# aifoundry-org/MHAQ

Measured on AMD Instinct MI355X. Metric: qat_images_per_sec, higher is better.
Workload: dtype f32; 1 GPU; ResNet-18 ImageNet-1k QAT step, AEWGS weights per-channel + STE activations, Sym-KL distillation from FP teacher, RAdam, synthetic 224x224, channels_last memory format; per_gpu_batch=250, global_batch=250, parallelism=dp1, sync_batchnorm=False, weight_backward_groups=3, cudnn_benchmark=False

## Files before the change

### mhaq_amd/csrc/torch_binding.cpp

```cpp
#include <torch/extension.h>
#include <torch/version.h>
#include <torch/csrc/autograd/custom_function.h>

#include <c10/hip/HIPCachingAllocator.h>
#include <c10/hip/HIPGraphsC10Utils.h>
#include <c10/hip/HIPStream.h>
#include <c10/core/DeviceGuard.h>
#include <dlfcn.h>

#include <algorithm>
#include <atomic>
#include <chrono>
#include <cstring>
#include <map>
#include <memory>
#include <mutex>
#include <string>
#include <unordered_map>
#include <vector>

#include "../../include/mhaq_fq.h"

namespace py = pybind11;
using at::Tensor;
// ... 756 lines not shown
    variable_list out(9);
    if (!grads[0].defined()) return out;
    TORCH_CHECK(!(at::GradMode::is_enabled() && grads[0].requires_grad()),
                "bn_pool_train: the node is once-differentiable (no double backward)");
    at::NoGradGuard no_grad;
    auto saved = ctx->get_saved_variables();
    const Tensor &x = saved[0], &w = saved[1], &mean = saved[2], &invstd = saved[3], &code = saved[4];
    const std::array<bool, 3> mask = {ctx->needs_input_grad(0), ctx->needs_input_grad(1), ctx->needs_input_grad(2)};
    Tensor g = grads[0].scalar_type() == at::kFloat ? grads[0] : grads[0].to(at::kFloat);
    if (g.sizes() != code.sizes() || g.strides() != code.strides()) {
      Tensor dense = at::empty_like(code, code.options().dtype(at::kFloat));
      dense.copy_(g);
      g = dense;
    }
    return bn_hip_backward(9, x, g, code, w, mean, invstd, mask);
  }
};

Tensor bn_pool_train(const Tensor& x, const std::optional<Tensor>& w, const std::optional<Tensor>& b,
                     const std::optional<Tensor>& running_mean, const std::optional<Tensor>& running_var, double momentum,
                     double eps, bool cudnn_enabled, bool hip_forward) {
  TORCH_CHECK(w.has_value() && w->defined() && b.has_value() && b->defined(),
              "bn_pool_train: an affine BatchNorm (weight and bias) is required");
  MHAQ_ON_DEVICE_OF(x);
  const bool hipf = hip_forward && bn_hip_forward_eligible(x, *w, *b, opt_tensor(running_mean), opt_tensor(running_var));
  if (!(bn_hip_eligible(x, *w) && x.scalar_type() == at::kFloat && x.numel() / x.size(1) < (1ll << 31)))
    return at::max_pool2d(BatchNormTrainFn::apply(x, w, b, running_mean, running_var, momentum, eps, cudnn_enabled,
                                                  false, hipf),
                          {3, 3}, {2, 2}, {1, 1});
  need_lib();
  return BatchNormPoolTrainFn::apply(x, *w, *b, running_mean, running_var, momentum, eps, cudnn_enabled, hipf);
}

struct Pre {
  bool has = false;
  Tensor wq, s, zp, mx, lwq;
};

PyObject* g_allreduce_avg = nullptr;
std::atomic<bool> g_dist_active{false};

void allreduce_avg(const Tensor& t) {
  py::gil_scoped_acquire gil;
  if (!g_allreduce_avg) throw MhaqError("AEWGS statistics exchange requested but no all-reduce is installed");
  py::reinterpret_borrow<py::object>(g_allreduce_avg)(t);
}

class WeightLayerFn : public torch::autograd::Function<WeightLayerFn> {
 public:
  static variable_list forward(AutogradContext* ctx, const Tensor& w, const Tensor& log_s, int64_t method,
                               const std::optional<Tensor>& r_sign, bool zp_grad, const Pre& pre, int64_t rank,
                               bool distributed) {
    const int64_t co = w.size(0), row = co ? w.numel() / co : 0;
    Tensor wq, s, zp, mx, lwq;
    if (pre.has) {
      wq = pre.wq; s = pre.s; zp = pre.zp; mx = pre.mx; lwq = pre.lwq;
    } else {
      wq = at::empty_like(w);
      Tensor aux = at::empty({4, co}, w.options());
      s = aux.select(0, 0); zp = aux.select(0, 1); mx = aux.select(0, 2); lwq = aux.select(0, 3);
      check(A.mhaq_fq_wlayer_fwd(fptr(w), fptr_mut(wq), fptr(log_s), co, row, fptr_mut(s), fptr_mut(zp), fptr_mut(mx),
                                 fptr_mut(lwq), cur_stream(w)),
            "mhaq_fq_wlayer_fwd");
    }
    weight_save_ctx(ctx, {w, s, zp, mx}, r_sign, method, rank, log_s);
    ctx->saved_data["dist"] = distributed;
    if (!zp_grad) ctx->mark_non_differentiable({s, zp});
    return {wq, zp, s, lwq};
  }

  static variable_list backward(AutogradContext* ctx, variable_list grads) {
    auto saved = ctx->get_saved_variables();
    const Tensor &w = saved[0], &s = saved[1], &zp = saved[2], &mx = saved[3];
    const bool has_r = saved.size() > 4;
    const int64_t method = ctx->saved_data["method"].toInt();
    Tensor G = grads[0].defined() ? like_layout(grads[0], w) : at::zeros_like(w);
    Tensor gzp_extra = grads[1].defined() ? grads[1].contiguous() : Tensor();
    Tensor g_lwq = grads[3].defined() ? grads[3].contiguous() : Tensor();
    const int64_t co = w.size(0), row = co ? w.numel() / co : 0;
    Tensor stats;
    if (method == MHAQ_FQ_AEWGS && ctx->saved_data["dist"].toBool()) {
      stats = at::empty({3, co}, w.options());
      check(A.mhaq_fq_pc_aewgs_stats(fptr(w), fptr(G), fptr(s), fptr(zp), co, row, fptr_mut(stats), cur_stream(w)),
            "mhaq_fq_pc_aewgs_stats");
      allreduce_avg(stats);
    }
    Tensor gw = at::empty_like(w);
    Tensor gls = at::empty({co}, w.options());
    const Draw d = draw_signs(has_r, method, ctx->saved_data["rank"].toInt(), w);
    check(A.mhaq_fq_wlayer_bwd(fptr(w), fptr(G), fptr_mut(gw), fptr_mut(gls), fptr(s), fptr(zp), fptr(mx),
                               fptr_or_null(g_lwq), co, row, (int)method, fptr_or_null(stats), fptr_or_null(gzp_extra),
                               saved_sign(saved, 4), d.seed, d.offset, d.offset_dev, cur_stream(w)),
          "mhaq_fq_wlayer_bwd");
    if (grads[2].defined())
      gls = gls + at::mul(at::mul(grads[2].reshape({co}), s), 0.69314718055994531);
    variable_list out(8);
    out[0] = gw;
    out[1] = ls_view(ctx, gls);
    return out;
  }
};

std::tuple<Tensor, Tensor, Tensor, Tensor> weight_layer(const Tensor& w_in, const Tensor& log_s_in, int64_t method,
                                                        const std::optional<Tensor>& r_sign, bool zp_grad,
                                                        const std::optional<std::vector<Tensor>>& pre, int64_t rank) {
  need_lib();
// ... 9 lines not shown
  if (pre.has_value()) {
    TORCH_CHECK(pre->size() >= 5, "weight_layer: pre = (wq, s, zp, mx, lwq[, s and zp in the published shape])");
    p.has = true;
    p.wq = (*pre)[0]; p.s = (*pre)[1]; p.zp = (*pre)[2]; p.mx = (*pre)[3]; p.lwq = (*pre)[4];
  }
  auto out = WeightLayerFn::apply(w, log_s, method, r_sign, zp_grad, p, rank, g_dist_active.load());
  std::vector<int64_t> shp(w.dim(), 1);
  shp[0] = w.size(0);
  return {out[0], out[1].view(shp), out[2].view(shp), out[3]};
}

std::tuple<Tensor, Tensor, Tensor, Tensor> pt_result(const variable_list& out) {
  const Tensor& aux = out[1];
  return {out[0], aux.select(0, 1), aux.narrow(0, 0, 1), out[2]};
}

class WeightLayerPTFn : public torch::autograd::Function<WeightLayerPTFn> {
 public:
  static variable_list forward(AutogradContext* ctx, const Tensor& w, const Tensor& log_s, int64_t method,
                               const std::optional<Tensor>& r_sign, int64_t rank) {
    Tensor wq = at::empty_like(w);
    Tensor aux = at::empty({4}, w.options());
    check(A.mhaq_fq_wlayer_pt_fwd(fptr(w), fptr_mut(wq), fptr(log_s), w.numel(), fptr_mut(aux), cur_stream(w)),
          "mhaq_fq_wlayer_pt_fwd");
    Tensor lwq = aux.narrow(0, 3, 1).clone();
    weight_save_ctx(ctx, {w, aux}, r_sign, method, rank, log_s);
    ctx->mark_non_differentiable({aux});
    return {wq, aux, lwq};
  }

  static variable_list backward(AutogradContext* ctx, variable_list grads) {
    auto saved = ctx->get_saved_variables();
    const Tensor &w = saved[0], &aux = saved[1];
    const bool has_r = saved.size() > 2;
    const int64_t method = ctx->saved_data["method"].toInt();
    Tensor G = grads[0].defined() ? grads[0].contiguous() : at::zeros_like(w);
    Tensor g_lwq = grads[2].defined() ? grads[2].contiguous() : Tensor();
    Tensor gw = at::empty_like(w);
    Tensor gls = at::empty({1}, w.options());
    const Draw d = draw_signs(has_r, method, ctx->saved_data["rank"].toInt(), w);
    check(A.mhaq_fq_wlayer_pt_bwd(fptr(w), fptr(G), fptr_mut(gw), fptr_mut(gls), fptr(aux), fptr_or_null(g_lwq), w.numel(),
                                  (int)method, saved_sign(saved, 2), d.seed, d.offset, d.offset_dev, cur_stream(w)),
          "mhaq_fq_wlayer_pt_bwd");
    variable_list out(5);
    out[0] = gw;
    out[1] = ls_view(ctx, gls);
    return out;
  }
};

std::tuple<Tensor, Tensor, Tensor, Tensor> weight_layer_pt(const Tensor& w_in, const Tensor& log_s, int64_t method,
                                                           const std::optional<Tensor>& r_sign, int64_t rank) {
  need_lib();
  MHAQ_ON_DEVICE_OF(w_in);
  TORCH_CHECK(w_in.is_cuda() && w_in.scalar_type() == at::kFloat && log_s.is_cuda() &&
                  log_s.scalar_type() == at::kFloat && log_s.numel() == 1,
              "weight_layer_pt: weight and a one-element log_wght_s must be float32 device tensors");
  const Tensor w = w_in.contiguous();
  auto out = WeightLayerPTFn::apply(w, log_s, method, r_sign, rank);
  return pt_result(out);
}

class WeightLayerPTLFn : public torch::autograd::Function<WeightLayerPTLFn> {
 public:
  static variable_list forward(AutogradContext* ctx, const Tensor& w, const Tensor& log_s, int64_t method,
                               const std::optional<Tensor>& r_sign, int64_t rank, bool distributed) {
    Tensor wq = at::empty_like(w);
    Tensor aux = at::empty({7}, w.options());
    const size_t nb = A.mhaq_fq_wlayer_ptl_workspace_bytes(w.numel());
    Tensor ws = at::empty({(int64_t)nb}, w.options().dtype(at::kByte));
    check(A.mhaq_fq_wlayer_ptl_fwd(fptr(w), fptr_mut(wq), fptr(log_s), w.numel(), fptr_mut(aux), ws.mutable_data_ptr(), nb,
                                   cur_stream(w)),
          "mhaq_fq_wlayer_ptl_fwd");
    Tensor lwq = aux.narrow(0, 3, 1).clone();
    weight_save_ctx(ctx, {w, aux}, r_sign, method, rank, log_s);
    ctx->saved_data["dist"] = distributed;
    ctx->mark_non_differentiable({aux});
    return {wq, aux, lwq};
  }

  static variable_list backward(AutogradContext* ctx, variable_list grads) {
    auto saved = ctx->get_saved_variables();
    const Tensor &w = saved[0], &aux = saved[1];
    const bool has_r = saved.size() > 2;
    const int64_t method = ctx->saved_data["method"].toInt();
    Tensor G = grads[0].defined() ? like_layout(grads[0], w) : at::zeros_like(w);
    Tensor g_lwq = grads[2].defined() ? grads[2].contiguous() : Tensor();
    const int64_t n = w.numel();
    void* stream = cur_stream(w);
    Tensor stats;
    int64_t period = 0;
    if (method == MHAQ_FQ_AEWGS) {
      const int64_t co = w.size(0);
      period = n / co;
      stats = at::empty({3, period}, w.options());
      const size_t sb = A.mhaq_fq_pt_aewgs_colstats_workspace_bytes(co, period);
      Tensor sws = sb ? at::empty({(int64_t)sb}, w.options().dtype(at::kByte)) : Tensor();
      check(A.mhaq_fq_pt_aewgs_colstats(fptr(w), fptr(G), co, period, fptr(aux), fptr(aux) + 1, nullptr, nullptr,
                                        fptr_mut(stats), sb ? sws.mutable_data_ptr() : nullptr, sb, stream),
            "mhaq_fq_pt_aewgs_colstats");
      if (ctx->saved_data["dist"].toBool()) allreduce_avg(stats);
    }
    Tensor gw = at::empty_like(w);
    Tensor gls = at::empty({1}, w.options());
    const size_t nb = A.mhaq_fq_wlayer_ptl_workspace_bytes(n);
    Tensor ws = at::empty({(int64_t)nb}, w.options().dtype(at::kByte));
    const Draw d = draw_signs(has_r, method, ctx->saved_data["rank"].toInt(), w);
    check(A.mhaq_fq_wlayer_ptl_bwd(fptr(w), fptr(G), fptr_mut(gw), fptr_mut(gls), fptr(aux), fptr_or_null(g_lwq), n,
                                   (int)method, fptr_or_null(stats), period, saved_sign(saved, 2), d.seed, d.offset,
                                   d.offset_dev, ws.mutable_data_ptr(), nb, stream),
          "mhaq_fq_wlayer_ptl_bwd");
    variable_list out(6);
    out[0] = gw;
    out[1] = ls_view(ctx, gls);
    return out;
  }
// ... 191 lines not shown
    ctx->saved_data["plan"] = plan_id;
    ctx->saved_data["group"] = gi;
    ctx->saved_data["rank"] = rank;
    ctx->saved_data["dist"] = distributed;
    ctx->saved_data["aux"] = p->cur_aux;
    std::vector<std::vector<int64_t>> ls_shapes;
    variable_list ws(tensors.begin(), tensors.begin() + n);
    for (int64_t k = 0; k < n; ++k) ls_shapes.push_back(tensors[n + k].sizes().vec());
    ctx->saved_data["ls_shapes"] = ls_shapes;
    ctx->save_for_backward(ws);
    ctx->set_materialize_grads(false);
    variable_list outs;
    outs.reserve(2 * n);
    for (int64_t k = 0; k < n; ++k) {
      const int64_t i = grp.first + k;
      outs.push_back(at::as_strided(p->cur_wq, ws[k].sizes(), ws[k].strides(), p->elem_off[i]));
    }
    for (int64_t k = 0; k < n; ++k) {
      const int64_t i = grp.first + k;
      outs.push_back(p->cur_aux.select(0, 3).narrow(0, p->chan_off[i], p->co[i]));
    }
    return outs;
  }

  static variable_list backward(AutogradContext* ctx, variable_list grads) {
    auto p = g_plans.get(ctx->saved_data["plan"].toInt());
    std::unique_lock<std::mutex> lk(p->mu);
    Group& grp = p->groups.at(ctx->saved_data["group"].toInt());
    const int64_t n = grp.n;
    auto ws = ctx->get_saved_variables();
    const Tensor aux_all = ctx->saved_data["aux"].toTensor();
    const Tensor& like = aux_all;
    void* stream = cur_stream(like);
    std::vector<Tensor> Gs(n), gl(n);
    for (int64_t k = 0; k < n; ++k) {
      Gs[k] = grads[k].defined() ? like_layout(grads[k], ws[k]) : at::zeros_like(ws[k]);
      if (grads[n + k].defined()) gl[k] = grads[n + k].contiguous();
    }
    if (!grp.pool) grp.pool = std::make_unique<TablePool>(sizeof(mhaq_wlayer_desc) * n, like);
    std::vector<int64_t> key;
    key.reserve(3 * n);
    for (int64_t k = 0; k < n; ++k) key.push_back((int64_t)(uintptr_t)ws[k].const_data_ptr());
    for (int64_t k = 0; k < n; ++k) key.push_back((int64_t)(uintptr_t)Gs[k].const_data_ptr());
    for (int64_t k = 0; k < n; ++k) key.push_back(gl[k].defined() ? (int64_t)(uintptr_t)gl[k].const_data_ptr() : 0);
    const Tensor table = grp.pool->get(key, [&](void* dst) {
      auto* d = static_cast<mhaq_wlayer_desc*>(dst);
      for (int64_t k = 0; k < n; ++k) {
        const int64_t i = grp.first + k;
        d[k] = mhaq_wlayer_desc{fptr(ws[k]), nullptr, fptr(Gs[k]), fptr_or_null(gl[k]), p->co[i], p->row[i],
                                p->elem_off[i] - grp.elem0, p->chan_off[i] - grp.chan0};
      }
    }, stream);
    const auto* descs = static_cast<const mhaq_wlayer_desc*>(table.const_data_ptr());
    const float* aux = fptr(aux_all) + grp.chan0;
    Tensor stats;
    if (grp.method == MHAQ_FQ_AEWGS && ctx->saved_data["dist"].toBool()) {
      stats = at::empty({3, grp.co}, like.options());
      check(A.mhaq_fq_wlayer_aewgs_stats_group(descs, (int)n, grp.co, aux, p->total_co, fptr_mut(stats), stream),
            "mhaq_fq_wlayer_aewgs_stats_group");
      lk.unlock();
      allreduce_avg(stats);
      lk.lock();
    }
    Tensor gw = at::empty({grp.elems}, like.options());
    Tensor gls = at::empty({grp.co}, like.options());
    const Draw d = draw_signs(false, grp.method, ctx->saved_data["rank"].toInt(), like);
// ... 145 lines not shown
    auto h = g_hubs.get(id);
    std::lock_guard<std::mutex> g(h->mu);
    py::dict d;
    d["tables"] = h->tables.entries.size();
    d["captured_tables"] = h->tables.captured();
    d["retired"] = h->retired.size();
    d["pending"] = h->pending.size();
    d["has_table"] = h->last_table.defined();
    int64_t bytes = 0;
    for (auto& w : h->ws) if (w.defined()) bytes += w.numel();
    for (auto& w : h->retired) bytes += w.numel();
    d["workspace_bytes"] = bytes;
    return d;
  });
  m.def("act_layer", &act_layer, py::arg("x"), py::arg("log_act_s"), py::arg("log_act_q"), py::arg("act_b"),
        py::arg("method"), py::arg("r_sign") = py::none(), py::arg("hub") = 0, py::arg("slot") = 0, py::arg("rank") = 0);
  m.def("act_relu_layer", &act_relu_layer, py::arg("z"), py::arg("addend"), py::arg("log_act_s"), py::arg("log_act_q"),
        py::arg("act_b"), py::arg("method"), py::arg("want_act"), py::arg("hub") = 0, py::arg("slot") = 0,
        py::arg("rank") = 0);

  m.def("bn_train", &bn_train, py::arg("x"), py::arg("weight"), py::arg("bias"), py::arg("running_mean"),
        py::arg("running_var"), py::arg("momentum"), py::arg("eps"), py::arg("cudnn_enabled") = true,
        py::arg("x16") = false, py::arg("hip_forward") = false);
  m.def("bn_hip_forwards", []() { return g_bn_hip_forwards.load(); },
        "number of BatchNorm forwards so far (bn_train and bn_pool_train) that ran mhaq_fq_bn_fwd instead of the framework's");

  m.def("bn_hip_backwards", []() { return g_bn_hip_backwards.load(); },
        "number of BatchNorm backwards so far that ran the fp32 HIP kernels instead of the framework's backward");
  m.def("bn_hip_backwards_x16", []() { return g_bn_hip_backwards_x16.load(); },
        "number of BatchNorm backwards so far that ran the 16-bit HIP kernels (mhaq_fq_bn_bwd_x16)");
  m.def("bn_pool_train", &bn_pool_train, py::arg("x"), py::arg("weight"), py::arg("bias"), py::arg("running_mean"),
        py::arg("running_var"), py::arg("momentum"), py::arg("eps"), py::arg("cudnn_enabled") = true,
        py::arg("hip_forward") = false);
  m.def("bn_pool_hip_backwards", []() { return g_bn_pool_hip_backwards.load(); },
        "number of BatchNorm + pool backwards so far that ran mhaq_fq_bn_pool_bwd (the fallback is the two separate nodes)");

  m.def("weight_layer", &weight_layer, py::arg("w"), py::arg("log_wght_s"), py::arg("method"),
        py::arg("r_sign") = py::none(), py::arg("zp_grad") = false, py::arg("pre") = py::none(), py::arg("rank") = 0);
  m.def("weight_layer_pt", &weight_layer_pt, py::arg("w"), py::arg("log_wght_s"), py::arg("method"),
        py::arg("r_sign") = py::none(), py::arg("rank") = 0);
  m.def("weight_layer_ptl", &weight_layer_ptl, py::arg("w"), py::arg("log_wght_s"), py::arg("method"),
        py::arg("r_sign") = py::none(), py::arg("rank") = 0);

  m.def("plan_create", &plan_create);
  m.def("plan_destroy", [](int64_t id) { g_plans.erase(id); });
  m.def("plan_forward", &plan_forward);
  m.def("plan_group_apply", &plan_group_apply);
  m.def("plan_release_captured", [](int64_t id) {
    auto p = g_plans.get(id);
    std::lock_guard<std::mutex> g(p->mu);
    for (auto& grp : p->groups) if (grp.pool) grp.pool->release_captured();
    p->fwd_tables.release_captured();
  });
  m.def("plan_state", [](int64_t id) {
    auto p = g_plans.get(id);
    std::lock_guard<std::mutex> g(p->mu);
    py::dict d;
    d["fwd_tables"] = p->fwd_tables.entries.size();
    py::list pools;
    for (auto& grp : p->groups) {
      py::dict e;
      size_t used = 0, held = 0, size = 0;
      if (grp.pool) {
        size = grp.pool->keys.size();
        for (size_t i = 0; i < size; ++i) { used += grp.pool->used[i]; held += grp.pool->held[i]; }
      }
// ... 10 lines not shown
```

### mhaq_amd/layers.py

```python
from __future__ import annotations

from typing import Tuple

import torch
import torch.nn.functional as F
from torch import inf, nn

from . import ops
from .enums import QNMethod, QScheme
from .gdnsq import Quantizer


def _rnoise_ratio(m):
    if m.rand_noise:
        return m._noise_ratio
    z = getattr(m, "_zero_ratio", None)
    if z is None or z.device != m._noise_ratio.device:
        z = torch.zeros_like(m._noise_ratio)
        m._zero_ratio = z
    return z


class NoisyAct(nn.Module):
    def __init__(
        self,
        init_s=-10,
        init_q=10,
        signed=True,
        noise_ratio=1,
        disable=False,
        qnmethod: QNMethod = QNMethod.STE,
    ) -> None:
        super().__init__()
        self.disable = disable
        self.signed = signed
        zero_point = 0.0 if not signed else -torch.exp2(torch.tensor(init_q - 1).float())
        self._act_b = torch.tensor([zero_point]).float()
        self._log_act_s = torch.tensor([init_s]).float()
        self._log_act_q = torch.tensor([init_q]).float()
        self._noise_ratio = torch.tensor(noise_ratio)
        self.log_act_q = nn.Parameter(self._log_act_q, requires_grad=True)
        self.act_b = nn.Parameter(self._act_b, requires_grad=bool(signed))
        self.log_act_s = nn.Parameter(self._log_act_s, requires_grad=True)
# ... 79 lines not shown
        self.Q.zero_point = self.act_b
        self.Q.min_val = self.act_b
        self.Q.max_val = params[3:4]

    def __getstate__(self):
        state = self.__dict__.copy()
        state.pop("_hub", None)
        return state

    def _forward_unfused_params(self, x):
        s = torch.exp2(self.log_act_s)
        q = torch.exp2(self.log_act_q)
        self.Q.zero_point = self.act_b
        self.Q.min_val = self.act_b
        self.Q.max_val = self.act_b + q - s
        self.Q.scale = s
        if self.training:
            return self.Q.fake_quant(x)
        y, qstats, _ = self.Q.fake_quant_eval(x)
        self.bw = torch.log2(qstats[1] - qstats[0] + 1)
        return y


class _WeightQuantMixin:
    quant_bias = False

    def _quantized_weight(self):
        d = self.__dict__
        self.Q.rnoise_ratio.data = _rnoise_ratio(self)
        weight_p, log_s_p = self.weight, self.log_wght_s
        grad_on = torch.is_grad_enabled()
        key = (weight_p._version, log_s_p._version, grad_on)
        pre = d.get("_precomputed")
        if pre is not None:
            d["_precomputed"] = None
            weight, zp, s, lwq, pkey = pre
            if pkey == key:
                d["_lwq"], d["_lwq_key"] = lwq, key
                self.Q.scale, self.Q.zero_point = s, zp
                return weight, s, zp
        per_channel = self.qscheme == QScheme.PER_CHANNEL
        if per_channel and self.quant_bias:
            weight, zp, s, lwq = ops.fake_quant_weight_layer(weight_p, log_s_p, self.Q.qnmethod, zp_grad=True)
            d["_lwq"], d["_lwq_key"] = lwq, key
        elif per_channel:
            pre = d.get("_pre_fwd")
            group = None
            if pre is not None:
                d["_pre_fwd"] = None
                group = pre[2]
                pre = pre[0] if pre[1] == (key[0], key[1], weight_p.data_ptr()) else None
            if pre is not None and group is not None and grad_on:
                weight, lwq = group[0].take(group[1])
                s, zp = pre[5], pre[6]
            else:
                weight, zp, s, lwq = ops.fake_quant_weight_layer(weight_p, log_s_p, self.Q.qnmethod, pre=pre)
            d["_lwq"], d["_lwq_key"] = lwq, key
        elif ops.small_pt_layer_supported(weight_p, self.Q.qnmethod):
            pre = d.get("_pre_fwd")
            group = None
            if pre is not None:
                d["_pre_fwd"] = None
                ok = pre[1] == (key[0], key[1], weight_p.data_ptr())
                group = pre[2]
                pre = pre[0] if (ok and group is not None and grad_on) else None
            if pre is not None:
                weight, lwq = group[0].take(group[1])
                zp, s = pre[2].reshape(()), pre[1]
            else:
                weight, zp, s, lwq = ops.fake_quant_weight_layer_pt(weight_p, log_s_p, self.Q.qnmethod)
            d["_lwq"], d["_lwq_key"] = lwq, key
        else:
            weight, zp, s, lwq = ops.fake_quant_weight_layer_ptl(weight_p, log_s_p, self.Q.qnmethod)
            d["_lwq"], d["_lwq_key"] = lwq, key
        self.Q.scale = s
        self.Q.zero_point = zp
        return weight, s, zp

    def regulariser_input(self):
        d = self.__dict__
        lwq = d.get("_lwq")
        if lwq is not None and d.get("_lwq_key") == (self.weight._version, self.log_wght_s._version,
                                                     torch.is_grad_enabled()):
            return lwq
        return None

    def __getstate__(self):
        state = self.__dict__.copy()
        for k in ("_pre_fwd", "_precomputed", "_lwq", "_lwq_key", "_zero_ratio"):
            state.pop(k, None)
        return state


class NoisyConv2d(_WeightQuantMixin, nn.Conv2d):
    def __init__(
        self,
        in_channels: int,
        out_channels: int,
        kernel_size: int | Tuple[int, int],
        stride: int | Tuple[int, int] = 1,
        padding: str | int | Tuple[int, int] = 0,
        dilation: int | Tuple[int, int] = 1,
        groups: int = 1,
        bias: bool = True,
        padding_mode: str = "zeros",
        device=None,
        dtype=None,
        qscheme: QScheme = QScheme.PER_TENSOR,
        log_s_init: float = -12,
        rand_noise: bool = False,
        quant_bias: bool = False,
        qnmethod: QNMethod = QNMethod.AEWGS,
    ) -> None:
        super().__init__(in_channels, out_channels, kernel_size, stride, padding, dilation, groups,
                         bias, padding_mode, device, dtype)
        self.qscheme = QScheme(qscheme.value) if not isinstance(qscheme, QScheme) else qscheme

        if self.qscheme == QScheme.PER_TENSOR:
            self.log_wght_s = nn.Parameter(torch.Tensor([log_s_init]), requires_grad=True)
        elif self.qscheme == QScheme.PER_CHANNEL:
            self.log_wght_s = nn.Parameter(
                torch.empty((out_channels, 1, 1, 1)).fill_(log_s_init), requires_grad=True)
            self.log_b_s = nn.Parameter(torch.empty(1).fill_(log_s_init), requires_grad=True)
        self._noise_ratio = nn.Parameter(torch.Tensor([1]), requires_grad=False)
        self.Q = Quantizer(self, torch.exp2(self.log_wght_s), 0, -inf, inf, qnmethod=qnmethod)
        self.rand_noise = rand_noise
        self.quant_bias = quant_bias
        if self.quant_bias:
            self.Q_b = Quantizer(self, torch.exp2(self.log_b_s), 0, -inf, inf, qnmethod=qnmethod)

    def forward(self, input: torch.Tensor) -> torch.Tensor:
        weight, s, zp = self._quantized_weight()
        if self.quant_bias:
            self.Q_b.scale = s.ravel()
            self.Q_b.zero_point = zp.ravel()
            self.Q_b.rnoise_ratio.data = _rnoise_ratio(self)
            bias = ops.fake_quant_per_element(self.bias, self.Q_b.scale, self.Q_b.zero_point,
                                              self.Q_b.qnmethod)
        else:
            bias = self.bias
        return self._conv_forward(input, weight, bias)

    def extra_repr(self) -> str:
        ls = self.log_wght_s.detach()
        grid = f"log_wght_s[{ls.numel()}] in [{float(ls.min()):.3f}, {float(ls.max()):.3f}]"
        return (f"{super().extra_repr()}, qscheme={self.qscheme.name}, estimator={getattr(self.Q.qnmethod, 'name', self.Q.qnmethod)}, "
                f"{grid}, quant_bias={self.quant_bias}, rand_noise={self.rand_noise}")


class NoisyLinear(_WeightQuantMixin, nn.Linear):
    def __init__(
        self,
        in_features: int,
        out_features: int,
        bias: bool = True,
        device=None,
        dtype=None,
        qscheme: QScheme = QScheme.PER_TENSOR,
        log_s_init: float = -12,
        rand_noise: bool = False,
        qnmethod: QNMethod = QNMethod.STE,
    ) -> None:
        super().__init__(in_features, out_features, bias, device, dtype)
        self.qscheme = QScheme(qscheme.value) if not isinstance(qscheme, QScheme) else qscheme
        if self.qscheme == QScheme.PER_TENSOR:
            self.log_wght_s = nn.Parameter(torch.Tensor([log_s_init]), requires_grad=True)
        elif self.qscheme == QScheme.PER_CHANNEL:
            self.log_wght_s = nn.Parameter(
                torch.empty((out_features, 1, 1, 1)).fill_(log_s_init), requires_grad=True)
        self._noise_ratio = nn.Parameter(torch.Tensor([1, ]), requires_grad=False)
        self.Q = Quantizer(self, torch.exp2(self.log_wght_s), 0, -inf, inf, qnmethod=qnmethod)
        self.rand_noise = rand_noise

    def forward(self, input: torch.Tensor) -> torch.Tensor:
# ... 9 lines not shown
```

### mhaq_amd/ops.py

```python
from __future__ import annotations

import contextlib
import functools
import ctypes
import math
import os

import torch
import torch.distributed as dist

from . import _lib
from ._ext import ext as _ext
from .enums import QNMethod

_MASK64 = (1 << 64) - 1
_i32 = ctypes.c_int32
_byref = ctypes.byref


_rank_cache = [None, 0]


def _rank() -> int:
    if not dist.is_available():
# ... 237 lines not shown
    w = _require_cuda_f32(w.detach(), "weight", any_dense_layout=True)
    co = w.shape[0]
    mn = torch.empty(co, dtype=torch.float32, device=w.device)
    mx = torch.empty(co, dtype=torch.float32, device=w.device)
    if co:
        _lib.check(_lib.lib().mhaq_fq_row_minmax(w.data_ptr(), co, w.numel() // co, mn.data_ptr(), mx.data_ptr(),
                                                 _stream()), "mhaq_fq_row_minmax")
    return mn, mx


@_on_device
def bn_forward_train(x, weight=None, bias=None, running_mean=None, running_var=None, factor=0.1, eps=1e-5):
    x = _require_cuda_f32(x.detach(), "x", any_dense_layout=True)
    if x.dim() != 4 or not x.is_contiguous(memory_format=torch.channels_last):
        raise ValueError("bn_forward_train: x must be a dense channels_last [N, C, H, W] tensor")
    c = x.shape[1]
    m = x.numel() // max(c, 1)
    vecs = [None if t is None else _require_cuda_f32(t.detach(), "a per-channel vector")
            for t in (weight, bias, running_mean, running_var)]
    if any(t is not None and (t.numel() != c or t.device != x.device) for t in vecs):
        raise ValueError("bn_forward_train: per-channel vectors must have C elements on x's device")
    if any(t is not None and t.data_ptr() != o.data_ptr() for t, o in zip(vecs[2:], (running_mean, running_var))):
        raise ValueError("bn_forward_train: the running statistics must be contiguous (they are updated in place)")
    L = _lib.lib()
    y = torch.empty_like(x)
    mean, invstd = torch.empty(c, device=x.device), torch.empty(c, device=x.device)
    nb = L.mhaq_fq_bn_fwd_workspace_bytes(m, c)
    ws = _workspace(max(nb, 16), x.device)
    ptr = lambda t: None if t is None else t.data_ptr()
    _lib.check(L.mhaq_fq_bn_fwd(x.data_ptr(), *map(ptr, vecs[:2]), y.data_ptr(), mean.data_ptr(), invstd.data_ptr(),
                                *map(ptr, vecs[2:]), float(factor), float(eps), m, c, ws.data_ptr(), nb, _stream()),
               "mhaq_fq_bn_fwd")
    return y, mean, invstd


def _pt_forward(x, s, zp, lo, hi, want_q=False, want_stats=False):
    L = _lib.lib()
    y = torch.empty_like(x)
    q = torch.empty_like(x) if want_q else None
    qstats = flags = ws = None
    nb = 0
    if want_stats:
        qstats = torch.empty(2, dtype=torch.float32, device=x.device)
        flags = torch.empty(1, dtype=torch.int32, device=x.device)
        nb = L.mhaq_fq_pt_fwd_workspace_bytes(x.numel())
        ws = _workspace(nb, x.device)
    _lib.check(L.mhaq_fq_pt_fwd(x.data_ptr(), y.data_ptr(), x.numel(), s.data_ptr(), zp.data_ptr(),
                                lo.data_ptr(), hi.data_ptr(), q.data_ptr() if want_q else None,
                                qstats.data_ptr() if want_stats else None,
                                flags.data_ptr() if want_stats else None,
                                ws.data_ptr() if ws is not None else None, nb, _stream()),
               "mhaq_fq_pt_fwd")
    return y, q, qstats, flags


def _pt_backward(x, g, s, zp, lo, hi, method, col_stats, period, r_sign, count_ties=False):
    L = _lib.lib()
    gx = torch.empty_like(x)
    grads = torch.empty(5, dtype=torch.float32, device=x.device)
    nb = L.mhaq_fq_pt_bwd_workspace_bytes(x.numel())
    ws = _workspace(nb, x.device)
    r_sign, seed, offset, odev = _signs(r_sign, method, x)
    _lib.check(L.mhaq_fq_pt_bwd(x.data_ptr(), g.data_ptr(), gx.data_ptr(), x.numel(), s.data_ptr(),
                                zp.data_ptr(), lo.data_ptr(), hi.data_ptr(), method,
                                col_stats.data_ptr() if col_stats is not None else None, period,
                                r_sign.data_ptr() if r_sign is not None else None, seed, offset, odev,
# ... 327 lines not shown
```

### mhaq_amd/qat.py

```python
from __future__ import annotations

import contextlib
import copy
import time
from dataclasses import dataclass, field
from typing import Optional

import torch
import torch.distributed as dist
from torch import nn

from . import ops
from ._lib import MhaqFqError
from .enums import QNMethod, QScheme
from .loss import FusedPotentialLoss, FusedPotentialLossNoPred, SymmetricalKL
from .wrap import get_model_values, quantize_model


@dataclass
class QATConfig:
    qscheme: QScheme = QScheme.PER_CHANNEL
    qnmethod: QNMethod = QNMethod.AEWGS
    act_bit: int = 1
    weight_bit: int = 1
    calib_act_bit: int = 10
    calib_weight_bit: int = 10
    excluded_layers: tuple = ("conv1", "fc")
    quantize_bias: bool = False
    distillation: bool = True
    learning_rate: float = 3e-4
    warmup: int = 100
    scale_lr: float = 1.0
    scale_t: float = 2.0
    sync_batchnorm: bool = True
    overlap_teacher: bool = True
    joint_act_finalize: bool = True
    student_high_priority: bool = False
    multi_weight_forward: bool = True
    weight_backward_group_elems: int = 4 << 20
    fuse_blocks: bool = True
    fuse_stem_pool: bool = True
    hip_bn_backward: bool = True
    hip_bn_backward_16bit: bool = False
    hip_bn_forward: bool = False
    criterion: nn.Module = field(default_factory=nn.CrossEntropyLoss)
    autocast_dtype: Optional[torch.dtype] = None


@torch.no_grad()
def calibrate_weights(model: nn.Module, wbits: int, max_bits: int = 24, row_minmax_fn=None) -> None:
    row_minmax_fn = row_minmax_fn or ops.row_minmax
    for m in model.modules():
        if hasattr(m, "log_wght_s") and hasattr(m, "weight"):
            mn, mx = row_minmax_fn(m.weight)
            mn, mx = mn.cpu(), mx.cpu()
            if m.log_wght_s.numel() == 1 and mn.numel() != 1:
                mn, mx = mn.min(), mx.max()
            if not m.log_wght_s.requires_grad:
                wbits = max_bits
            floor = torch.log2((mx - mn) / (2 ** wbits - 1)).reshape(m.log_wght_s.shape)
            m.log_wght_s.copy_(torch.max(m.log_wght_s.detach().cpu(), floor))


def _cpu_row_minmax(w):
    dims = tuple(range(1, w.dim()))
    return w.detach().amin(dims), w.detach().amax(dims)


@torch.no_grad()
def calibrate_activations(model: nn.Module, batches, abits: int, max_bits: int = 24, minmax_fn=None) -> None:
    minmax_fn = minmax_fn or ops.minmax
    acts = [m for m in model.modules() if hasattr(m, "log_act_s") and hasattr(m, "act_b")]
    seen = {id(a): [] for a in acts}
    hooks = [a.register_forward_pre_hook(lambda mod, inp: seen[id(mod)].append(minmax_fn(inp[0]))) for a in acts]
    was_training = model.training
    model.eval()
    for x in batches:
# ... 68 lines not shown
            if self.act_hub is not None:
                self.act_hub.end()


class QATTrainer:
    def __init__(self, net: nn.Module, cfg: QATConfig, device, calib_batches=None, layers=None,
                 distributed=None, minmax_fn=None, optimizer_factory=None,
                 multi_tensor_weights=False, capture_graph=None, loss_classes=None):
        self.cfg, self.device = cfg, torch.device(device)
        if cfg.autocast_dtype is not None and cfg.autocast_dtype != torch.bfloat16:
            raise ValueError(f"QATConfig.autocast_dtype: {cfg.autocast_dtype} is not supported (None or torch.bfloat16; "
                             "float16 training needs loss scaling, which this trainer does not do)")
        self.distributed = ops._dist_active() if distributed is None else distributed
        net = net.to(self.device)
        self.teacher = copy.deepcopy(net).eval().requires_grad_(False) if cfg.distillation else None
        quantize_model(net, cfg.qscheme, cfg.qnmethod, cfg.excluded_layers, cfg.quantize_bias, cfg.act_bit,
                       layers=layers)
        net.to(self.device)
        if calib_batches is not None:
            calibrate_weights(net, cfg.calib_weight_bit,
                              row_minmax_fn=_cpu_row_minmax if self.device.type != "cuda" else None)
            calibrate_activations(net, calib_batches, cfg.calib_act_bit, minmax_fn=minmax_fn)
        if self.distributed and cfg.sync_batchnorm and self.device.type == "cuda":
            net = nn.SyncBatchNorm.convert_sync_batchnorm(net)
        if cfg.fuse_blocks and layers is None and self.device.type == "cuda":
            from . import fused_blocks
            if fused_blocks.enabled_by_env():
                fused_blocks.install(net, stem_pool=cfg.fuse_stem_pool and fused_blocks.stem_pool_enabled_by_env())
        if cfg.hip_bn_backward and layers is None and self.device.type == "cuda":
            from . import bn_backward
            if bn_backward.enabled_by_env():
                bn_backward.install(net, x16=bn_backward.x16_enabled(cfg.hip_bn_backward_16bit),
                                    hip_forward=bn_backward.hip_forward_enabled(cfg.hip_bn_forward))
        self.net = net
        self.teacher_stream = None
        if cfg.distillation and cfg.overlap_teacher and self.device.type == "cuda":
            self.teacher_stream = torch.cuda.Stream(device=self.device)
        self._hp_stream = None
        if cfg.student_high_priority and self.device.type == "cuda":
            self._hp_stream = torch.cuda.Stream(device=self.device, priority=-1)
        self.multi = None
        if multi_tensor_weights and self.distributed:
            raise ValueError("multi_tensor_weights is a single-GPU option (the data-parallel trainer keeps the "
                             "per-layer ops: AEWGS statistics all-reduce + gradient overlap)")
        if multi_tensor_weights:
            from .multi import MultiTensorWeightQuant
            self.multi = MultiTensorWeightQuant(net)
        self.act_hub = None
        if cfg.joint_act_finalize and self.device.type == "cuda" and (layers is None):
            from .act_hub import ActGradHub
            hub = ActGradHub(net)
            self.act_hub = hub if len(hub) > 1 else None
        self.weight_forward = None
        if cfg.multi_weight_forward and self.multi is None and self.device.type == "cuda" and layers is None:
            from .multi import MultiTensorWeightQuant
            try:
                wf = MultiTensorWeightQuant(net, joint_backward=False,
                                            backward_group_elems=cfg.weight_backward_group_elems)
                self.weight_forward = wf if wf.nlayers > 1 else None
            except ValueError:
                pass
        self.module = _QATModule(net, cfg.qscheme, self.act_hub, self.weight_forward)
        self._flat_sync = False
        want_capture = capture_graph
        if want_capture is None:
            want_capture = "auto" if (layers is None and optimizer_factory is None and not multi_tensor_weights) else False
# ... 236 lines not shown
            self._preflight_syncs = [str(w.message) for w in caught if is_sync(w)]
            for w in caught:
                if not is_sync(w) and "debug mode is a prototype" not in str(w.message):
                    warnings.warn_explicit(w.message, w.category, w.filename, w.lineno)
            return loss
        if not self.module.training:
            self.module.train()
        if not self.loss.training:
            self.loss.train()
        if self.multi is not None:
            self.multi.run()
        side = self.teacher_stream if self.cfg.distillation else None
        fp = None
        if side is not None:
            main = torch.cuda.current_stream()
            side.wait_stream(main)
            with torch.cuda.stream(side), torch.no_grad(), self._autocast():
                fp = self.teacher(x)
        with self._autocast():
            out = self.module(x)
            if self.cfg.distillation:
                if side is None:
                    with torch.no_grad():
                        fp = self.teacher(x)
                else:
                    main.wait_stream(side)
                    if not torch.cuda.is_current_stream_capturing():
                        fp.record_stream(main)
                loss = self.loss(out, fp)
            else:
                loss = self.loss((self.cfg.criterion(out[0], y), *out[1:]))
        self.optimizer.zero_grad(set_to_none=True)
        loss.backward()
        return loss

    @torch.no_grad()
    def validate_step(self, x, y):
        from . import stats
        from .gdnsq import check_model_integrity
        self.module.eval()
        try:
            with self._autocast():
                out = self.net(x)
            out = out.float()
            check_model_integrity(self.net)
        finally:
            self.module.train()
        with stats.memoised():
            return self._validation_record(out, y, stats)

    def _validation_record(self, out, y, stats):
        return {
            "val_loss": self.cfg.criterion(out, y),
            "top1": (out.argmax(1) == y).float().mean(),
            "mean_weights_bit_width": stats.get_weights_bit_width_mean(self.net),
            "actual_weights_bit_width": stats.get_true_weights_width(self.net, max=False),
            "actual_weights_max_bit_width": stats.get_true_weights_width(self.net),
            "mean_activations_bit_width": stats.get_activations_bit_width_mean(self.net),
            "actual_activations_bit_width": stats.get_true_activations_width(self.net, max=False),
            "actual_activations_max_bit_width": stats.get_true_activations_width(self.net),
            "converged": stats.is_converged(self.net, self.loss),
        }
```

Baseline: 6563 images/s.

## Add conv autograd node that can defer weight gradients to a side stream

Adds a compiled ConvTrainFn autograd node. It splits the conv backward into an input-gradient call and a separate weight-gradient call. When deferral is enabled, the weight gradient runs on a per-device side stream, and the fake-quant weight backward nodes and the end of the step join on that stream first. Deferral is off by default (config false, env unset), so the default path only replaces F.conv2d with the custom node and two convolution_backward calls instead of one. That adds per-layer overhead and may lose fused backward.

```diff
diff --git a/mhaq_amd/csrc/torch_binding.cpp b/mhaq_amd/csrc/torch_binding.cpp
--- a/mhaq_amd/csrc/torch_binding.cpp
+++ b/mhaq_amd/csrc/torch_binding.cpp
@@ -812,6 +812,135 @@
   return BatchNormPoolTrainFn::apply(x, *w, *b, running_mean, running_var, momentum, eps, cudnn_enabled, hipf);
 }
 
+struct WgradLane {
+  std::mutex mu;
+  std::optional<c10::hip::HIPStream> side;
+  hipEvent_t ev_main = nullptr, ev_side = nullptr;
+  int64_t pending = 0;
+};
+constexpr int kMaxLanes = 64;
+std::array<WgradLane, kMaxLanes>& g_lanes = *new std::array<WgradLane, kMaxLanes>();
+std::atomic<int64_t> g_wgrad_deferred{0};
+std::atomic<int64_t> g_wgrad_inline{0};
+
+inline WgradLane& wgrad_lane(int64_t device) {
+  TORCH_CHECK(device >= 0 && device < kMaxLanes, "weight-gradient lane: device index ", device, " out of range");
+  return g_lanes[(size_t)device];
+}
+
+c10::hip::HIPStream wgrad_side_locked(WgradLane& lane, int64_t device) {
+  if (!lane.side.has_value()) {
+    lane.side = c10::hip::getStreamFromPool(false, (c10::DeviceIndex)device);
+    C10_HIP_CHECK(hipEventCreateWithFlags(&lane.ev_main, hipEventDisableTiming));
+    C10_HIP_CHECK(hipEventCreateWithFlags(&lane.ev_side, hipEventDisableTiming));
+  }
+  return *lane.side;
+}
+
+void wgrad_join(int64_t device) {
+  WgradLane& lane = wgrad_lane(device);
+  std::lock_guard<std::mutex> g(lane.mu);
+  if (lane.pending == 0 || capturing()) return;
+  const c10::OptionalDeviceGuard device_guard(c10::Device(c10::kCUDA, (c10::DeviceIndex)device));
+  const auto cur = c10::hip::getCurrentHIPStream((c10::DeviceIndex)device);
+  if (cur != *lane.side) {
+    C10_HIP_CHECK(hipEventRecord(lane.ev_side, lane.side->stream()));
+    C10_HIP_CHECK(hipStreamWaitEvent(cur.stream(), lane.ev_side, 0));
+  }
+  lane.pending = 0;
+}
+
+inline void wgrad_join_for(const Tensor& t) {
+  if (t.defined() && t.is_cuda()) wgrad_join(t.device().index());
+}
+
+struct CurrentStreamSwitch {
+  c10::hip::HIPStream prev;
+  CurrentStreamSwitch(c10::hip::HIPStream prev_, c10::hip::HIPStream next) : prev(prev_) { c10::hip::setCurrentHIPStream(next); }
+  ~CurrentStreamSwitch() { c10::hip::setCurrentHIPStream(prev); }
+};
+
+class ConvTrainFn : public torch::autograd::Function<ConvTrainFn> {
+ public:
+  static Tensor forward(AutogradContext* ctx, const Tensor& x, const Tensor& w, const std::optional<Tensor>& bias,
+                        std::vector<int64_t> stride, std::vector<int64_t> padding, std::vector<int64_t> dilation,
+                        int64_t groups, bool defer) {
+    const bool has_b = bias.has_value() && bias->defined();
+    Tensor y = at::convolution(x, w, bias, stride, padding, dilation, false, {0, 0}, groups);
+    ctx->save_for_backward({x, w});
+    if (has_b) ctx->saved_data["bias_sizes"] = bias->sizes().vec();
+    ctx->saved_data["stride"] = stride;
+    ctx->saved_data["padding"] = padding;
+    ctx->saved_data["dilation"] = dilation;
+    ctx->saved_data["groups"] = groups;
+    ctx->saved_data["defer"] = defer;
+    ctx->set_materialize_grads(false);
+    return y;
+  }
+
+  static variable_list backward(AutogradContext* ctx, const variable_list& grads) {
+    variable_list out(8);
+    if (!grads[0].defined()) return out;
+    TORCH_CHECK(!at::GradMode::is_enabled(), "conv_train: the node is once-differentiable (no double backward)");
+    auto saved = ctx->get_saved_variables();
+    const Tensor &x = saved[0], &w = saved[1], &dy = grads[0];
+    const auto stride = ctx->saved_data["stride"].toIntVector(), padding = ctx->saved_data["padding"].toIntVector(),
+               dilation = ctx->saved_data["dilation"].toIntVector();
+    const int64_t groups = ctx->saved_data["groups"].toInt();
+    std::vector<int64_t> bias_sizes;
+    const bool has_b = ctx->saved_data.count("bias_sizes") != 0;
+    if (has_b) bias_sizes = ctx->saved_data["bias_sizes"].toIntVector();
+    const at::OptionalIntArrayRef bsz = has_b ? at::OptionalIntArrayRef(bias_sizes) : at::OptionalIntArrayRef();
+    const std::array<bool, 3> first = {ctx->needs_input_grad(0), false, has_b && ctx->needs_input_grad(2)};
+    auto direction = [&](const std::array<bool, 3>& mask) {
+      return at::convolution_backward(dy, x, w, bsz, stride, padding, dilation, false, {0, 0}, groups, mask);
+    };
+    if (first[0] || first[2]) {
+      auto g = direction(first);
+      if (first[0]) out[0] = std::get<0>(g);
+      if (first[2]) out[2] = std::get<2>(g);
+    }
+    if (!ctx->needs_input_grad(1)) return out;
+    const std::array<bool, 3> second = {false, true, false};
+    if (!dy.is_cuda()) {
+      out[1] = std::get<1>(direction(second));
+      return out;
+    }
+    const int64_t device = dy.device().index();
+    const auto main = c10::hip::getCurrentHIPStream((c10::DeviceIndex)device);
+    const bool own_dy = dy.use_count() == 1 && dy.storage().use_count() == 1;
+    if (ctx->saved_data["defer"].toBool() && own_dy && !capturing()) {
+      WgradLane& lane = wgrad_lane(device);
+      std::lock_guard<std::mutex> g(lane.mu);
+      const auto side = wgrad_side_locked(lane, device);
+      if (side != main) {
+        C10_HIP_CHECK(hipEventRecord(lane.ev_main, main.stream()));
+        C10_HIP_CHECK(hipStreamWaitEvent(side.stream(), lane.ev_main, 0));
+        Tensor dw;
+        {
+          CurrentStreamSwitch on_side(main, side);
+          dw = std::get<1>(direction(second));
+        }
+        ++lane.pending;
+        for (const Tensor* t : {&dy, &x, &w}) c10::hip::HIPCachingAllocator::recordStream(t->storage().data_ptr(), side);
+        if (dw.defined()) c10::hip::HIPCachingAllocator::recordStream(dw.storage().data_ptr(), main);
+        g_wgrad_deferred.fetch_add(1, std::memory_order_relaxed);
+        out[1] = dw;
+        return out;
+      }
+    }
+    out[1] = std::get<1>(direction(second));
+    g_wgrad_inline.fetch_add(1, std::memory_order_relaxed);
+    return out;
+  }
+};
+
+Tensor conv_train(const Tensor& x, const Tensor& w, const std::optional<Tensor>& bias, std::vector<int64_t> stride,
+                  std::vector<int64_t> padding, std::vector<int64_t> dilation, int64_t groups, bool defer) {
+  MHAQ_ON_DEVICE_OF(x);
+  return ConvTrainFn::apply(x, w, bias, std::move(stride), std::move(padding), std::move(dilation), groups, defer);
+}
+
 struct Pre {
   bool has = false;
   Tensor wq, s, zp, mx, lwq;
@@ -852,6 +981,7 @@
   static variable_list backward(AutogradContext* ctx, variable_list grads) {
     auto saved = ctx->get_saved_variables();
     const Tensor &w = saved[0], &s = saved[1], &zp = saved[2], &mx = saved[3];
+    wgrad_join_for(w);
     const bool has_r = saved.size() > 4;
     const int64_t method = ctx->saved_data["method"].toInt();
     Tensor G = grads[0].defined() ? like_layout(grads[0], w) : at::zeros_like(w);
@@ -927,6 +1057,7 @@
   static variable_list backward(AutogradContext* ctx, variable_list grads) {
     auto saved = ctx->get_saved_variables();
     const Tensor &w = saved[0], &aux = saved[1];
+    wgrad_join_for(w);
     const bool has_r = saved.size() > 2;
     const int64_t method = ctx->saved_data["method"].toInt();
     Tensor G = grads[0].defined() ? grads[0].contiguous() : at::zeros_like(w);
@@ -977,6 +1108,7 @@
   static variable_list backward(AutogradContext* ctx, variable_list grads) {
     auto saved = ctx->get_saved_variables();
     const Tensor &w = saved[0], &aux = saved[1];
+    wgrad_join_for(w);
     const bool has_r = saved.size() > 2;
     const int64_t method = ctx->saved_data["method"].toInt();
     Tensor G = grads[0].defined() ? like_layout(grads[0], w) : at::zeros_like(w);
@@ -1234,6 +1366,7 @@
     const Tensor aux_all = ctx->saved_data["aux"].toTensor();
     const Tensor& like = aux_all;
     void* stream = cur_stream(like);
+    wgrad_join_for(like);
     std::vector<Tensor> Gs(n), gl(n);
     for (int64_t k = 0; k < n; ++k) {
       Gs[k] = grads[k].defined() ? like_layout(grads[k], ws[k]) : at::zeros_like(ws[k]);
@@ -1445,6 +1578,22 @@
   m.def("bn_pool_train", &bn_pool_train, py::arg("x"), py::arg("weight"), py::arg("bias"), py::arg("running_mean"),
         py::arg("running_var"), py::arg("momentum"), py::arg("eps"), py::arg("cudnn_enabled") = true,
         py::arg("hip_forward") = false);
+  m.def("conv_train", &conv_train, py::arg("x"), py::arg("weight"), py::arg("bias"), py::arg("stride"), py::arg("padding"),
+        py::arg("dilation"), py::arg("groups"), py::arg("defer") = false,
+        "F.conv2d as a compiled node; defer: run the weight gradient on the device's weight-gradient lane (its consumer "
+        "must call wgrad_join first)");
+  m.def("wgrad_join", &wgrad_join, py::arg("device"),
+        "make the current stream of `device` wait for the weight gradients issued on its lane since the last join");
+  m.def("wgrad_stream", [](int64_t device) {
+    WgradLane& lane = wgrad_lane(device);
+    std::lock_guard<std::mutex> g(lane.mu);
+    const c10::OptionalDeviceGuard device_guard(c10::Device(c10::kCUDA, (c10::DeviceIndex)device));
+    return (uintptr_t)wgrad_side_locked(lane, device).stream();
+  }, py::arg("device"), "the raw stream handle of the device's weight-gradient lane (created on first use)");
+  m.def("wgrad_deferred", []() { return g_wgrad_deferred.load(); },
+        "how many device weight gradients conv_train has issued on a weight-gradient lane");
+  m.def("wgrad_inline", []() { return g_wgrad_inline.load(); },
+        "how many device weight gradients conv_train has issued on the current stream");
   m.def("bn_pool_hip_backwards", []() { return g_bn_pool_hip_backwards.load(); },
         "number of BatchNorm + pool backwards so far that ran mhaq_fq_bn_pool_bwd (the fallback is the two separate nodes)");
 
diff --git a/mhaq_amd/layers.py b/mhaq_amd/layers.py
--- a/mhaq_amd/layers.py
+++ b/mhaq_amd/layers.py
@@ -1,5 +1,6 @@
 from __future__ import annotations
 
+import os
 from typing import Tuple
 
 import torch
@@ -9,6 +10,26 @@
 from . import ops
 from .enums import QNMethod, QScheme
 from .gdnsq import Quantizer
+
+
+ENV_WGRAD_OVERLAP = "MHAQ_WGRAD_OVERLAP"
+OVERLAP_WGRAD = "_mhaq_overlap_wgrad"
+
+
+def overlap_wgrad_enabled(configured: bool = False) -> bool:
+    v = os.environ.get(ENV_WGRAD_OVERLAP)
+    if v is None or not v.strip():
+        return bool(configured)
+    return v.strip().lower() in ("1", "true", "on", "yes")
+
+
+def install_overlap_wgrad(net, on: bool = True) -> int:
+    n = 0
+    for m in net.modules():
+        if isinstance(m, NoisyConv2d):
+            m.__dict__[OVERLAP_WGRAD] = bool(on)
+            n += 1
+    return n
 
 
 def _rnoise_ratio(m):
@@ -154,6 +175,7 @@
         grad_on = torch.is_grad_enabled()
         key = (weight_p._version, log_s_p._version, grad_on)
         pre = d.get("_precomputed")
+        d["_wq_joins"] = False
         if pre is not None:
             d["_precomputed"] = None
             weight, zp, s, lwq, pkey = pre
@@ -161,6 +183,7 @@
                 d["_lwq"], d["_lwq_key"] = lwq, key
                 self.Q.scale, self.Q.zero_point = s, zp
                 return weight, s, zp
+        d["_wq_joins"] = True
         per_channel = self.qscheme == QScheme.PER_CHANNEL
         if per_channel and self.quant_bias:
             weight, zp, s, lwq = ops.fake_quant_weight_layer(weight_p, log_s_p, self.Q.qnmethod, zp_grad=True)
@@ -209,7 +232,7 @@
 
     def __getstate__(self):
         state = self.__dict__.copy()
-        for k in ("_pre_fwd", "_precomputed", "_lwq", "_lwq_key", "_zero_ratio"):
+        for k in ("_pre_fwd", "_precomputed", "_lwq", "_lwq_key", "_zero_ratio", "_wq_joins", OVERLAP_WGRAD):
             state.pop(k, None)
         return state
 
@@ -261,7 +284,19 @@
                                               self.Q_b.qnmethod)
         else:
             bias = self.bias
+        if self._takes_conv_node(input, weight):
+            d = self.__dict__
+            return ops.conv_train(input, weight, bias, self.stride, self.padding, self.dilation, self.groups,
+                                  defer=bool(d.get(OVERLAP_WGRAD) and d.get("_wq_joins")))
         return self._conv_forward(input, weight, bias)
+
+    def _takes_conv_node(self, input, weight) -> bool:
+        if "_conv_forward" in self.__dict__ or type(self)._conv_forward is not nn.Conv2d._conv_forward:
+            return False
+        return (not self.quant_bias and self.padding_mode == "zeros" and not isinstance(self.padding, str)
+                and input.is_cuda and input.dim() == 4 and input.dtype == torch.float32 and weight.dtype == torch.float32
+                and not torch.is_autocast_enabled("cuda") and torch.is_grad_enabled()
+                and (input.requires_grad or weight.requires_grad))
 
     def extra_repr(self) -> str:
         ls = self.log_wght_s.detach()
diff --git a/mhaq_amd/ops.py b/mhaq_amd/ops.py
--- a/mhaq_amd/ops.py
+++ b/mhaq_amd/ops.py
@@ -293,6 +293,35 @@
                                 *map(ptr, vecs[2:]), float(factor), float(eps), m, c, ws.data_ptr(), nb, _stream()),
                "mhaq_fq_bn_fwd")
     return y, mean, invstd
+
+
+def conv_train(x, weight, bias=None, stride=1, padding=0, dilation=1, groups=1, defer=False):
+    pair = lambda v: [int(v), int(v)] if isinstance(v, int) else [int(e) for e in v]
+    return _ext().conv_train(x, weight, bias, pair(stride), pair(padding), pair(dilation), int(groups), bool(defer))
+
+
+def _device_index(device=None) -> int:
+    if device is None:
+        return torch.cuda.current_device()
+    device = torch.device(device)
+    return torch.cuda.current_device() if device.index is None else device.index
+
+
+def wgrad_join(device=None) -> None:
+    _ext().wgrad_join(_device_index(device))
+
+
+def wgrad_stream(device=None):
+    idx = _device_index(device)
+    return torch.cuda.ExternalStream(_ext().wgrad_stream(idx), device=torch.device("cuda", idx))
+
+
+def wgrad_deferred() -> int:
+    return _ext().wgrad_deferred()
+
+
+def wgrad_inline() -> int:
+    return _ext().wgrad_inline()
 
 
 def _pt_forward(x, s, zp, lo, hi, want_q=False, want_stats=False):
diff --git a/mhaq_amd/qat.py b/mhaq_amd/qat.py
--- a/mhaq_amd/qat.py
+++ b/mhaq_amd/qat.py
@@ -43,6 +43,7 @@
     hip_bn_backward: bool = True
     hip_bn_backward_16bit: bool = False
     hip_bn_forward: bool = False
+    overlap_wgrad: bool = False
     criterion: nn.Module = field(default_factory=nn.CrossEntropyLoss)
     autocast_dtype: Optional[torch.dtype] = None
 
@@ -177,6 +178,11 @@
             if bn_backward.enabled_by_env():
                 bn_backward.install(net, x16=bn_backward.x16_enabled(cfg.hip_bn_backward_16bit),
                                     hip_forward=bn_backward.hip_forward_enabled(cfg.hip_bn_forward))
+        self.overlap_wgrad = False
+        if layers is None and self.device.type == "cuda":
+            from . import layers as hip_layers
+            self.overlap_wgrad = hip_layers.overlap_wgrad_enabled(cfg.overlap_wgrad)
+            hip_layers.install_overlap_wgrad(net, self.overlap_wgrad)
         self.net = net
         self.teacher_stream = None
         if cfg.distillation and cfg.overlap_teacher and self.device.type == "cuda":
@@ -479,6 +485,8 @@
                 loss = self.loss((self.cfg.criterion(out[0], y), *out[1:]))
         self.optimizer.zero_grad(set_to_none=True)
         loss.backward()
+        if self.device.type == "cuda":
+            ops.wgrad_join(self.device)
         return loss
 
     @torch.no_grad()
```

Measured after the change: 6534 images/s. No clear change (-0.5%).
